# KIT-MBS/pydca

Measured on AMD Instinct MI355X. Metric: plmDCA L-BFGS iterations/s (L=500 N=50000 q=21), higher is better.
Workload: dtype f32

## Files before the change

pydca_amd/csrc/lbfgs_kernels.h:

```cpp
#pragma once

#include "dca_internal.h"
#include "plm_plan.h"
#include "vec_kernels.h"

namespace {

template <bool DD> struct DotAcc;
template <> struct DotAcc<false> {
    double hi = 0.0;
    static constexpr double lo = 0.0;
    __device__ __forceinline__ void add(double a, double b) { hi += a * b; }
    __device__ __forceinline__ void wave_reduce() { for (int off = 32; off > 0; off >>= 1) hi += __shfl_down(hi, off); }
};
template <> struct DotAcc<true> {
    double hi = 0.0, lo = 0.0;
    __device__ __forceinline__ void add(double a, double b) { dd_add(hi, lo, __dmul_rn(a, b)); }
    __device__ __forceinline__ void wave_reduce() { dd_wave_reduce(hi, lo); }
};
template <int NV>
__device__ __forceinline__ void dot_block_store(double (*red)[2 * NV], int nv, double* __restrict__ partials, unsigned grid = 0)
{
    __syncthreads();
    if ((int)threadIdx.x < nv) {
// ... 174 lines not shown
        if (e < (size_t)L * Q) {
            T sv[5], yv[5];
#pragma unroll
            for (int k = 0; k < 5; ++k) { sv[k] = static_cast<const T*>(P.s[k])[e]; yv[k] = static_cast<const T*>(P.y[k])[e]; }
            const T dv = compose_elem(c, g[e], sv, yv);
            d[e] = dv;
            const T v = one * dv;
            xt[e] = x[e] + v;
        }
        return;
    }
    const int blk = ((int)blockIdx.x & ~63) | (((int)blockIdx.x & 7) << 3) | (((int)blockIdx.x >> 3) & 7);
    if (blk >= pairBlocks) return;
    const int i0 = (blk / numJC) * TI, j0 = (blk % numJC) * JC;
    const int j1 = min(j0 + JC, L);
    if (j1 <= i0 + 1) return;
    if (tid == 0) {
        int pre = 0;
        for (int ii = 0; ii < TI; ++ii) {
            const int i = i0 + ii, jlo = max(j0, i + 1);
            const int cnt = jlo < j1 ? (j1 - jlo) * Q2 : 0;
            const size_t before = (size_t)L * (L - 1) / 2 - (size_t)(L - i) * (L - i - 1) / 2;
            const size_t lo = cnt ? (size_t)L * Q + (before + (size_t)(jlo - i - 1)) * Q2 : 0;
            sLo[ii] = lo; sCnt[ii] = cnt; sPre[ii] = pre;
            pre += cnt ? (int)((lo + cnt + VEC - 1) / VEC - lo / VEC) : 0;
        }
        sPre[TI] = pre;
    }
    __syncthreads();
    const int total = sPre[TI];
    for (int idx = tid; idx < total; idx += kFusedStepThreads) {
        int ii = 0;
        while (idx >= sPre[ii + 1]) ++ii;
        const size_t lo = sLo[ii], hi = lo + (size_t)sCnt[ii];
        const size_t iv = lo / VEC + (size_t)(idx - sPre[ii]);
        const Pack<T> pg = ldp_at(g, iv); const Pack<T> px = ldp_at(x, iv);
        Pack<T> psk[5]; Pack<T> pyk[5];
#pragma unroll
        for (int k = 0; k < 5; ++k) { psk[k] = ldp_at(static_cast<const T*>(P.s[k]), iv); pyk[k] = ldp_at(static_cast<const T*>(P.y[k]), iv); }
        Pack<T> od, ox;
#pragma unroll
        for (int u = 0; u < VEC; ++u) {
            T sv[5], yv[5];
#pragma unroll
            for (int k = 0; k < 5; ++k) { sv[k] = psk[k].v[u]; yv[k] = pyk[k].v[u]; }
            od.v[u] = compose_elem(c, pg.v[u], sv, yv);
            const T v = one * od.v[u];
            ox.v[u] = px.v[u] + v;
        }
        const size_t e0 = iv * VEC;
        T* const dst = tile + (size_t)(ii * JC + (max(j0, i0 + ii + 1) - j0)) * Q2;
        if (e0 >= lo && e0 + VEC <= hi) {
            stp_at(d, iv, od); stp_at(xt, iv, ox);
#pragma unroll
            for (int u = 0; u < VEC; ++u) dst[e0 + u - lo] = ox.v[u];
        } else {
#pragma unroll
            for (int u = 0; u < VEC; ++u) {
                const size_t e = e0 + u;
                if (e >= lo && e < hi) { d[e] = od.v[u]; xt[e] = ox.v[u]; dst[e - lo] = ox.v[u]; }
            }
        }
    }
    __syncthreads();
    {
        constexpr int WD = JC * Q;
        int row = tid / WD, col = tid % WD;
        while (row < TI * Q) {
            const int ii = row / Q, jj = col / Q;
            const int i = i0 + ii, j = j0 + jj;
            if (j > i && j < j1) W[(size_t)(i0 * Q + row) * Cs + j0 * Q + col] = tile[row * Q + ii * ((JC - 1) * Q2) + col + jj * ((Q - 1) * Q)];
            row += kFusedStepThreads / WD; col += kFusedStepThreads % WD;
            if (col >= WD) { col -= WD; ++row; }
        }
    }
    {
        constexpr int WD = TI * Q;
        int row = tid / WD, col = tid % WD;
        while (row < JC * Q) {
            const int jj = row / Q, ii = col / Q;
            const int i = i0 + ii, j = j0 + jj;
            if (j > i && j < j1) W[(size_t)(j0 * Q + row) * Cs + i0 * Q + col] = tile[col * Q + ii * ((JC - 1) * Q2) + row + jj * ((Q - 1) * Q)];
            row += kFusedStepThreads / WD; col += kFusedStepThreads % WD;
            if (col >= WD) { col -= WD; ++row; }
        }
    }
}

__global__ __launch_bounds__(256)
void vec_final_kernel(const double* __restrict__ partials, int nb, int nk, double* __restrict__ out)
{
    __shared__ double redHi[256], redLo[256];
    const int k = blockIdx.x;
    double hi = 0.0, lo = 0.0;
    for (int b = threadIdx.x; b < nb; b += blockDim.x) dd_add2(hi, lo, partials[2 * ((size_t)k * nb + b)], partials[2 * ((size_t)k * nb + b) + 1]);
    dd_block_reduce(hi, lo, redHi, redLo);
    if (threadIdx.x == 0) out[k] = hi + lo;
}

__global__ __launch_bounds__(256)
void dd_sum_chunks_kernel(const double* __restrict__ parts, int n, double* __restrict__ out)
{
    __shared__ double redHi[256], redLo[256];
    const int chunk = (n + gridDim.x - 1) / gridDim.x;
    const int lo_ = blockIdx.x * chunk, hi_ = min(n, lo_ + chunk);
    double hi = 0.0, lo = 0.0;
    for (int b = lo_ + threadIdx.x; b < hi_; b += blockDim.x) dd_add2(hi, lo, parts[2 * (size_t)b], parts[2 * (size_t)b + 1]);
    dd_block_reduce(hi, lo, redHi, redLo);
    if (threadIdx.x == 0) { out[2 * blockIdx.x] = hi; out[2 * blockIdx.x + 1] = lo; }
}
__global__ __launch_bounds__(1024)
void dd_sum_final_kernel(const double* __restrict__ A, int nA, const double* __restrict__ B, int nB, double* __restrict__ out)
{
    __shared__ double redHi[1024], redLo[1024];
    double hi = 0.0, lo = 0.0;
    for (int b = threadIdx.x; b < nA; b += blockDim.x) dd_add2(hi, lo, A[2 * (size_t)b], A[2 * (size_t)b + 1]);
    for (int b = threadIdx.x; b < nB; b += blockDim.x) dd_add2(hi, lo, B[2 * (size_t)b], B[2 * (size_t)b + 1]);
    dd_block_reduce(hi, lo, redHi, redLo);
    if (threadIdx.x == 0) out[0] = hi + lo;
}

template <typename T>
__global__ __launch_bounds__(kVecThreads)
void vec_dot3_fx_kernel(const T* __restrict__ a, const T* __restrict__ b, const T* __restrict__ c, size_t n, double* __restrict__ partials,
                        const double* __restrict__ fxParts, int nFxParts, double* __restrict__ fxChunks)
{
    if (blockIdx.x >= (unsigned)kVecBlocks) {
        __shared__ double redHi[256], redLo[256];
        const int blk = (int)blockIdx.x - kVecBlocks;
        const int chunk = (nFxParts + kSumStageBlocks - 1) / kSumStageBlocks;
        const int lo_ = blk * chunk, hi_ = min(nFxParts, lo_ + chunk);
        double hi = 0.0, lo = 0.0;
        for (int p = lo_ + threadIdx.x; p < hi_; p += blockDim.x) dd_add2(hi, lo, fxParts[2 * (size_t)p], fxParts[2 * (size_t)p + 1]);
        dd_block_reduce(hi, lo, redHi, redLo);
        if (threadIdx.x == 0) { fxChunks[2 * blk] = hi; fxChunks[2 * blk + 1] = lo; }
        return;
    }
    __shared__ double red[kVecThreads / 64][6];
    DotAcc<sizeof(T) == 8> s0, s1, s2;
    DCA_VEC_LOOP_G(n, a, kVecBlocks,
        const Pack<T> pa = ldp_at(a + head_, iv); const Pack<T> pb = ldp_at(b + head_, iv); const Pack<T> pc = ldp_at(c + head_, iv);
        _Pragma("unroll") for (int k = 0; k < VEC; ++k) {
            const double av = pa.v[k]; const double bv = pb.v[k]; const double cv = pc.v[k];
            s0.add(av, bv); s1.add(cv, cv); s2.add(av, av);
        },
        { const double av = a[i]; const double bv = b[i]; const double cv = c[i]; s0.add(av, bv); s1.add(cv, cv); s2.add(av, av); })
    s0.wave_reduce(); s1.wave_reduce(); s2.wave_reduce();
    if ((threadIdx.x & 63) == 0) {
        double* r = red[threadIdx.x >> 6];
        r[0] = s0.hi; r[1] = s0.lo; r[2] = s1.hi; r[3] = s1.lo; r[4] = s2.hi; r[5] = s2.lo;
    }
    dot_block_store<3>(red, 3, partials, kVecBlocks);
}
__global__ __launch_bounds__(1024)
void vec_final_fx_kernel(const double* __restrict__ partials, int nb, int nk, double* __restrict__ out,
                         const double* __restrict__ A, int nA, const double* __restrict__ B, int nB, double* __restrict__ fxOut)
{
    __shared__ double redHi[1024], redLo[1024];
    const int k = blockIdx.x;
    double hi = 0.0, lo = 0.0;
    if (k < nk) {
        constexpr int NT = 256;
        if ((int)threadIdx.x < NT) {
            for (int b = threadIdx.x; b < nb; b += NT) dd_add2(hi, lo, partials[2 * ((size_t)k * nb + b)], partials[2 * ((size_t)k * nb + b) + 1]);
            redHi[threadIdx.x] = hi;
            redLo[threadIdx.x] = lo;
        }
        __syncthreads();
        for (int st = NT / 2; st > 0; st >>= 1) {
            if ((int)threadIdx.x < st) dd_add2(redHi[threadIdx.x], redLo[threadIdx.x], redHi[threadIdx.x + st], redLo[threadIdx.x + st]);
            __syncthreads();
        }
        if (threadIdx.x == 0) out[k] = redHi[0] + redLo[0];
        return;
    }
    for (int b = threadIdx.x; b < nA; b += blockDim.x) dd_add2(hi, lo, A[2 * (size_t)b], A[2 * (size_t)b + 1]);
    for (int b = threadIdx.x; b < nB; b += blockDim.x) dd_add2(hi, lo, B[2 * (size_t)b], B[2 * (size_t)b + 1]);
    dd_block_reduce(hi, lo, redHi, redLo);
    if (threadIdx.x == 0) fxOut[0] = hi + lo;
}

}
```

pydca_amd/csrc/plm_engine.hip:

```cpp
#include <algorithm>
#include <chrono>
#include <cmath>

#include "dca_internal.h"
#include "more_thuente.h"
#include "vec_kernels.h"
#include "plm_plan.h"
#include "plm_stages.h"
#include "lbfgs_kernels.h"

namespace {

static_assert(kPlanXcds == kNumXcd, "the planner deals strips to this many XCDs");

#ifdef DCA_ROUND_ABLATE
__global__ void round_to_f32_kernel(double* __restrict__ p, size_t n)
{
    for (size_t i = blockIdx.x * (size_t)blockDim.x + threadIdx.x; i < n; i += (size_t)gridDim.x * blockDim.x) p[i] = (double)(float)p[i];
}
inline int round_stage_mask() { const char* e = getenv("DCA_ROUND_F32_STAGES"); return e ? atoi(e) : 0; }
#define DCA_ROUND_STAGE(bit, ptr, count)                                                                             \
    do {                                                                                                             \
        if constexpr (sizeof(T) == 8)                                                                                \
            if (round_stage_mask() & (bit))                                                                          \
                hipLaunchKernelGGL(round_to_f32_kernel, dim3(2048), dim3(256), 0, ctx->stream, reinterpret_cast<double*>(ptr), (size_t)(count)); \
    } while (0)
#else
#define DCA_ROUND_STAGE(bit, ptr, count) do { } while (0)
#endif

template <typename T>
struct PlmEngine : PlmEngineBase {
    dca_ctx* ctx;
    int N, L, q, Ls;
    double lambda_h = 0, lambda_J = 0;
    int carry_mode = DCA_CARRY_CHUNKED, halo = 0, add_reg = 1;
    bool configured = false;
    PlmPlan plan;
    PlmKnobs knobs;

    T *dx = nullptr, *dg = nullptr, *dxp = nullptr, *dgp = nullptr, *dd = nullptr;
    T* dS[5] = {nullptr, nullptr, nullptr, nullptr, nullptr};
    T* dY[5] = {nullptr, nullptr, nullptr, nullptr, nullptr};
    T *dWt = nullptr, *dSR = nullptr, *dR = nullptr, *dG = nullptr, *dw = nullptr;
    LbfgsDev* dLb = nullptr;
    uint16_t* dXL = nullptr;
    uint16_t* dXT2 = nullptr;
    PairIJ* dPairs = nullptr;
    double *dFxPart = nullptr, *dRegPart = nullptr, *dVecPart = nullptr;
    double *dColPart = nullptr, *dColSum = nullptr;
    double* dColChunk = nullptr;
    bool stripRequested = false, strips = false, stripEmulate = false;
    int sWorld = 1, sRank = 0;
    T *dGrecv = nullptr, *dXsend = nullptr, *dXrecv = nullptr;
    template <typename F> void each_buffer(F f)
    {
        f(dx); f(dg); f(dxp); f(dgp); f(dd);
        for (int i = 0; i < 5; ++i) { f(dS[i]); f(dY[i]); }
        f(dWt); f(dSR); f(dR); f(dG); f(dw); f(dLb); f(dXL); f(dXT2); f(dPairs); f(dFxPart); f(dRegPart); f(dVecPart);
        f(dColPart); f(dColSum); f(dColChunk); f(dGrecv); f(dXsend); f(dXrecv);
    }
    int strip_cs(int r) const { return plm_strip_cs(plan.siteB, q, r); }
    size_t owned_lo(int r) const { return plm_owned_lo(plan.siteB, L, q, r); }
    size_t owned_hi(int r) const { return plm_owned_hi(plan.siteB, L, q, r); }
    bool lbfgs_alloc = false;
    bool deferFx = false, fxPending = false;
    size_t vlo = 0, vn = 0, Ppad = 0;
    dca_comm_hook comm = nullptr;
    void* comm_user = nullptr;
    int comm_rank = 0, comm_world = 0;

    struct {
        bool begun = false, finished = false;
        int status = 0, k = 1, end = 0, iters = 0, evals = 0, max_iterations = 0, verbose = 0;
        double fx = 0, step = 0, xnorm = 0, gnorm = 0, seconds = 0;
        double last_step = 0;
        double dginit = 0;
        bool dginit_on_device = false;
        bool trial_ready = false;
    } o;

    explicit PlmEngine(dca_ctx* c) : ctx(c), N(c->N), L(c->L), q(c->q), Ls(c->Ls) {}

    template <typename U> int dalloc(U** p, size_t n)
    {
        HIP_TRY(dca_dev_malloc(reinterpret_cast<void**>(p), std::max<size_t>(n, 1) * sizeof(U)));
        return DCA_OK;
    }
    void freeall() { each_buffer([](auto*& p) { dca_dev_free(p); p = nullptr; }); }
    ~PlmEngine() override { freeall(); }

    void weights_changed() override { configured = false; o = decltype(o)(); }

    int configure(double lh, double lJ, int cmode, int chunk_, int warm_, int halo_, int add_reg_) override
    {
        if (q != 21 && q != 5) { dca_set_error("plmDCA kernels are built for q = 21 (protein) and q = 5 (RNA); got %d", q); return DCA_ERR_ARG; }
        if (!ctx->have_weights) { dca_set_error("weights must be computed or set before dca_plm_configure"); return DCA_ERR_STATE; }
        if (halo_ < 0 || halo_ >= N) { dca_set_error("halo out of range"); return DCA_ERR_ARG; }
        if (L > 65535) { dca_set_error("L too large"); return DCA_ERR_ARG; }
        configured = false;
        lambda_h = lh; lambda_J = lJ; carry_mode = cmode; halo = halo_; add_reg = add_reg_;
        strips = stripRequested && ctx->comm && ctx->comm_world > 1;
        stripRequested = false;
        sWorld = strips ? ctx->comm_world : 1;
        sRank = strips ? ctx->comm_rank : 0;
#ifdef DCA_ROUND_ABLATE
        stripEmulate = false;
        if (const char* e = getenv("DCA_STRIP_EMULATE")) {
            int er = 0, ew = 1;
            if (sscanf(e, "%d,%d", &er, &ew) == 2 && ew > 1 && er >= 0 && er < ew) { strips = true; stripEmulate = true; sRank = er; sWorld = ew; }
        }
#endif
        if (sWorld > kMaxStripRanks || (strips && sWorld > L)) { dca_set_error("column strips: too many ranks for %d sites", L); return DCA_ERR_ARG; }
        if (strips && (halo || hook || comm)) { dca_set_error("column strips take the whole alignment and no hooks"); return DCA_ERR_ARG; }
        knobs = PlmKnobs::from_env();
        PlmShape shape;
        shape.N = N; shape.L = L; shape.q = q; shape.elemBytes = (int)sizeof(T); shape.halo = halo; shape.chunkArg = chunk_; shape.warmArg = warm_;
        shape.carryMode = carry_mode; shape.stripWorld = sWorld; shape.stripRank = sRank; shape.strips = strips;
        plan = plm_make_plan(shape, knobs, PlmKernelShapes{{logits_seq_per_wg(5), logits_seq_per_wg(21), logits_seq_per_wg(kPairQ)},
                                                           {logits_jt(5), logits_jt(21), logits_jt(kPairQ)}});
        const int Lq = L * q, JT = plan.JT;
        const size_t npairs = (size_t)L * (L - 1) / 2;

        freeall();
        lbfgs_alloc = false;
        o = decltype(o)();

        DCA_TRY(dalloc(&dx, plan.P + kVecPad)); DCA_TRY(dalloc(&dg, plan.P + kVecPad));
        DCA_TRY(dalloc(&dWt, (size_t)plan.Wrows * plan.Cs));
        DCA_TRY(dalloc(&dSR, (size_t)N * plan.Cs));
        DCA_TRY(dalloc(&dR, (size_t)(N + kNC) * plan.Cs));
        HIP_TRY(hipMemsetAsync(dR, 0, (size_t)(N + kNC) * plan.Cs * sizeof(T), ctx->stream));
        DCA_TRY(dalloc(&dG, plan.num_slabs() * plan.slab_elems()));
        DCA_TRY(dalloc(&dw, N));
        DCA_TRY(dalloc(&dXL, (size_t)ceil_div(plan.gUnits, JT) * JT * plan.Npad));
        DCA_TRY(dalloc(&dXT2, (size_t)plan.gUnits * plan.NT));
        DCA_TRY(dalloc(&dPairs, npairs));
        DCA_TRY(dalloc(&dFxPart, 2 * (size_t)plan.nFxPart));
        DCA_TRY(dalloc(&dRegPart, 2 * (size_t)(plan.nRegPart + kSumStageBlocks)));
        DCA_TRY(dalloc(&dVecPart, 2 * 27 * kVecBlocks));
        HIP_TRY(hipMemsetAsync(dRegPart, 0, 2 * (size_t)(plan.nRegPart + kSumStageBlocks) * sizeof(double), ctx->stream));
        HIP_TRY(hipMemsetAsync(dFxPart, 0, 2 * (size_t)plan.nFxPart * sizeof(double), ctx->stream));
        if (sizeof(T) == 8) {
            DCA_TRY(dalloc(&dColPart, 2 * (size_t)kColSumRowBlocks * Lq));
            if (q == 5) DCA_TRY(dalloc(&dColChunk, 2 * (size_t)plan.numScanChunks * Lq));
            DCA_TRY(dalloc(&dColSum, (size_t)Lq));
        }
        if (strips) { DCA_TRY(dalloc(&dGrecv, plan.grecvOff[sWorld])); DCA_TRY(dalloc(&dXsend, plan.xsendOff[sWorld])); DCA_TRY(dalloc(&dXrecv, plan.xrecvOff[sWorld])); }

        HIP_TRY(hipMemsetAsync(dx, 0, (plan.P + kVecPad) * sizeof(T), ctx->stream));
        HIP_TRY(hipMemsetAsync(dg, 0, (plan.P + kVecPad) * sizeof(T), ctx->stream));
        vlo = 0; vn = plan.P; Ppad = plan.P;
        if (strips) {
            native_mode = 4;
            vlo = plan.oLo; vn = plan.oHi - plan.oLo;
        } else if (native_mode == 4) {
            native_mode = 0;
        }
        if (native_mode == 2 || native_mode == 3) {
            if (!ctx->comm) native_mode = 0;
            else DCA_TRY(set_slices(ctx->comm_rank, ctx->comm_world));
        } else if (comm) {
            DCA_TRY(set_slices(comm_rank, comm_world));
        }
        if (native_mode == 1 && !ctx->comm) native_mode = 0;
        HIP_TRY(hipMemsetAsync(dWt, 0, (size_t)plan.Wrows * plan.Cs * sizeof(T), ctx->stream));
        HIP_TRY(hipMemsetAsync(dG, 0, plan.num_slabs() * plan.slab_elems() * sizeof(T), ctx->stream));

        std::vector<PairIJ> hp(npairs);
        {
            size_t k = 0;
            for (int i = 0; i < L - 1; ++i) for (int j = i + 1; j < L; ++j) hp[k++] = PairIJ{(uint16_t)i, (uint16_t)j};
        }
        HIP_TRY(hipMemcpyAsync(dPairs, hp.data(), npairs * sizeof(PairIJ), hipMemcpyHostToDevice, ctx->stream));
        HIP_TRY(hipStreamSynchronize(ctx->stream));

        std::vector<T> hw(N);
        {
            std::vector<double> wd(N);
            HIP_TRY(hipMemcpy(wd.data(), ctx->dWd, (size_t)N * sizeof(double), hipMemcpyDeviceToHost));
            if (ctx->have_counts) {
                std::vector<uint32_t> cnt(N);
                HIP_TRY(hipMemcpy(cnt.data(), ctx->dCounts, (size_t)N * sizeof(uint32_t), hipMemcpyDeviceToHost));
                for (int n = 0; n < N; ++n) hw[n] = (T)1 / (T)cnt[n];
            } else {
                for (int n = 0; n < N; ++n) hw[n] = (T)wd[n];
            }
        }
        HIP_TRY(hipMemcpy(dw, hw.data(), (size_t)N * sizeof(T), hipMemcpyHostToDevice));

        if (plan.pairs) {
            hipLaunchKernelGGL(plm_build_pair_states_kernel, dim3(ceil_div(plan.Npad, 256), ceil_div(plan.gUnits, JT) * JT), dim3(256), 0,
                               ctx->stream, ctx->dX, dXL, N, plan.Npad, L, Ls, 0, 0x2000u);
            hipLaunchKernelGGL(plm_build_pair_states_kernel, dim3(ceil_div(plan.NT, 256), plan.gUnits), dim3(256), 0, ctx->stream,
                               ctx->dX, dXT2, N, plan.NT, L, Ls, halo, 0x9000u);
            HIP_TRY(hipGetLastError());
            HIP_TRY(hipStreamSynchronize(ctx->stream));
        } else {
            hipLaunchKernelGGL(plm_build_logit_states_kernel, dim3(ceil_div(plan.Npad, 256), ceil_div(L, JT) * JT), dim3(256), 0,
                               ctx->stream, ctx->dX, dXL, N, plan.Npad, L, Ls);
            hipLaunchKernelGGL(plm_build_states_kernel, dim3(ceil_div(plan.NT, 256), L), dim3(256), 0, ctx->stream,
                               ctx->dX, dXT2, N, L, Ls, halo, plan.NT);
            HIP_TRY(hipGetLastError());
            HIP_TRY(hipStreamSynchronize(ctx->stream));
        }
        configured = true;
        return DCA_OK;
    }

    int configure_strips(double lh, double lJ, int cmode, int chunk_, int warm_) override
    {
        if (!ctx->comm) { dca_set_error("column strips need a communicator: dca_comm_init first"); return DCA_ERR_STATE; }
        if (o.begun && !o.finished) { dca_set_error("the decomposition cannot change during an optimisation"); return DCA_ERR_STATE; }
        const auto hook0 = hook; const auto hookUser0 = hook_user; const auto comm0 = comm; const auto commUser0 = comm_user;
        const int commRank0 = comm_rank, commWorld0 = comm_world;
        hook = nullptr; hook_user = nullptr; comm = nullptr; comm_user = nullptr; comm_rank = comm_world = 0;
        stripRequested = true;
        const int rc = configure(lh, lJ, cmode, chunk_, warm_, 0, 1);
        stripRequested = false;
        if (rc != DCA_OK) { hook = hook0; hook_user = hookUser0; comm = comm0; comm_user = commUser0; comm_rank = commRank0; comm_world = commWorld0; strips = false; }
        return rc;
    }

    int init_x() override
    {
        if (!configured) { dca_set_error("dca_plm_configure first"); return DCA_ERR_STATE; }
        std::vector<T> hw(N);
        HIP_TRY(hipMemcpy(hw.data(), dw, (size_t)N * sizeof(T), hipMemcpyDeviceToHost));
        T meff = 0;
        for (int n = 0; n < N; ++n) meff += hw[n];
        std::vector<T> h((size_t)L * q, (T)0);
        const uint8_t* X = dca_host_msa(ctx);
        if (!X) return DCA_ERR_HIP;
        for (int n = 0; n < N; ++n)
            for (int i = 0; i < L; ++i) h[(size_t)i * q + X[(size_t)n * L + i]] += hw[n];
        for (int i = 0; i < L; ++i) {
            T* hi = h.data() + (size_t)i * q;
            for (int a = 0; a < q; ++a) hi[a] /= meff;
            for (int a = 0; a < q; ++a) hi[a] = std::log(hi[a] * meff + (T)1);
            T s = 0;
            for (int a = 0; a < q; ++a) s += hi[a];
            const T av = s / (T)q;
            for (int a = 0; a < q; ++a) hi[a] -= av;
        }
        o.trial_ready = false;
        HIP_TRY(hipMemsetAsync(dx, 0, plan.P * sizeof(T), ctx->stream));
        HIP_TRY(hipMemcpyAsync(dx, h.data(), h.size() * sizeof(T), hipMemcpyHostToDevice, ctx->stream));
        HIP_TRY(hipStreamSynchronize(ctx->stream));
        return DCA_OK;
    }

    template <typename U> int upload(const U* src, T* dst)
    {
        std::vector<T> tmp(plan.P);
        for (size_t i = 0; i < plan.P; ++i) tmp[i] = (T)src[i];
        HIP_TRY(hipMemcpy(dst, tmp.data(), plan.P * sizeof(T), hipMemcpyHostToDevice));
        return DCA_OK;
    }
    template <typename U> int download(const T* src, U* dst)
    {
        std::vector<T> tmp(plan.P);
        HIP_TRY(hipStreamSynchronize(ctx->stream));
        HIP_TRY(hipMemcpy(tmp.data(), src, plan.P * sizeof(T), hipMemcpyDeviceToHost));
        for (size_t i = 0; i < plan.P; ++i) dst[i] = (U)tmp[i];
        return DCA_OK;
    }
    int set_x(const void* x, int dtype) override
    {
        if (!configured) { dca_set_error("dca_plm_configure first"); return DCA_ERR_STATE; }
        o.trial_ready = false;
        if (dtype == DCA_F32) return upload(static_cast<const float*>(x), dx);
        if (dtype == DCA_F64) return upload(static_cast<const double*>(x), dx);
        return DCA_ERR_ARG;
    }
    int get_x(void* x, int dtype) override
    {
        if (!configured) return DCA_ERR_STATE;
        if (native_mode == 4 && !stripEmulate) DCA_TRY(strip_allgather(dx));
        if (dtype == DCA_F32) return download(dx, static_cast<float*>(x));
        if (dtype == DCA_F64) return download(dx, static_cast<double*>(x));
        return DCA_ERR_ARG;
    }
    int get_g(void* g, int dtype) override
    {
        if (!configured) return DCA_ERR_STATE;
        DCA_TRY(gather_vector(dg));
        if (dtype == DCA_F32) return download(dg, static_cast<float*>(g));
        if (dtype == DCA_F64) return download(dg, static_cast<double*>(g));
        return DCA_ERR_ARG;
    }

    template <int Q> int launch_eval(bool w_ready)
    {
// ... 150 lines not shown
        if (native_mode == 4) return stripEmulate ? DCA_OK : strip_allgather(v);
        return do_comm(DCA_COMM_ALL_GATHER, v, Ppad, (int)sizeof(T) * 8, "all-gather");
    }
    int publish_x()
    {
        if (native_mode == 4) return stripEmulate ? DCA_OK : exchange_x();
        return gather_vector(dx);
    }

    int exchange_x()
    {
        const int dt = (int)sizeof(T) * 8;
        const size_t q2 = (size_t)q * q;
        for (int r = sRank + 1; r < sWorld; ++r) {
            const int ni = plan.siteB[r + 1] - plan.siteB[r];
            hipLaunchKernelGGL((strip_pairs_copy_kernel<T, true>), dim3((unsigned)(plan.Lloc * ni)), dim3(64), 0, ctx->stream, dx, dXsend + plan.xsendOff[r], L, q, plan.cS0, plan.cS1, plan.siteB[r], plan.siteB[r + 1]);
        }
        DCA_TRY(dca_comm_p2p_begin(ctx));
        int rc = DCA_OK;
        if (sRank == 0) { for (int r = 1; r < sWorld && rc == DCA_OK; ++r) rc = dca_comm_p2p_send(ctx, dx + (size_t)plan.siteB[r] * q, (size_t)(plan.siteB[r + 1] - plan.siteB[r]) * q, dt, r); }
        else rc = dca_comm_p2p_recv(ctx, dx + (size_t)plan.cS0 * q, (size_t)plan.Lloc * q, dt, 0);
        for (int r = sRank + 1; r < sWorld && rc == DCA_OK; ++r) rc = dca_comm_p2p_send(ctx, dXsend + plan.xsendOff[r], (size_t)plan.Lloc * (plan.siteB[r + 1] - plan.siteB[r]) * q2, dt, r);
        for (int r = 0; r < sRank && rc == DCA_OK; ++r) rc = dca_comm_p2p_recv(ctx, dXrecv + plan.xrecvOff[r], (size_t)(plan.siteB[r + 1] - plan.siteB[r]) * plan.Lloc * q2, dt, r);
        const int rc2 = dca_comm_p2p_end(ctx);
        if (rc != DCA_OK) return rc;
        DCA_TRY(rc2);
        for (int r = 0; r < sRank; ++r) {
            const int nj = plan.siteB[r + 1] - plan.siteB[r];
            hipLaunchKernelGGL((strip_pairs_copy_kernel<T, false>), dim3((unsigned)(nj * plan.Lloc)), dim3(64), 0, ctx->stream, dx, dXrecv + plan.xrecvOff[r], L, q, plan.siteB[r], plan.siteB[r + 1], plan.cS0, plan.cS1);
        }
        HIP_TRY(hipGetLastError());
        return DCA_OK;
    }
    int exchange_g()
    {
        const int dt = (int)sizeof(T) * 8;
        DCA_TRY(dca_comm_p2p_begin(ctx));
        int rc = DCA_OK;
        for (int r = 0; r < sRank && rc == DCA_OK; ++r)
            rc = dca_comm_p2p_send(ctx, dG + (size_t)plan.siteB[r] * q * plan.Cs, (size_t)(plan.siteB[r + 1] - plan.siteB[r]) * q * plan.Cs, dt, r);
        for (int r = sRank + 1; r < sWorld && rc == DCA_OK; ++r)
            rc = dca_comm_p2p_recv(ctx, dGrecv + plan.grecvOff[r], (size_t)plan.Lloc * q * strip_cs(r), dt, r);
        if (rc == DCA_OK) {
            if (sRank > 0) rc = dca_comm_p2p_send(ctx, dg + (size_t)plan.cS0 * q, (size_t)plan.Lloc * q, dt, 0);
            else for (int r = 1; r < sWorld && rc == DCA_OK; ++r) rc = dca_comm_p2p_recv(ctx, dg + (size_t)plan.siteB[r] * q, (size_t)(plan.siteB[r + 1] - plan.siteB[r]) * q, dt, r);
        }
        const int rc2 = dca_comm_p2p_end(ctx);
        if (rc != DCA_OK) return rc;
        return rc2;
    }
    int strip_allgather(T* v)
    {
        const int dt = (int)sizeof(T) * 8;
        DCA_TRY(dca_comm_p2p_begin(ctx));
        int rc = DCA_OK;
        for (int k = 1; k < sWorld && rc == DCA_OK; ++k) {
            const int to = (sRank + k) % sWorld, from = (sRank - k + sWorld) % sWorld;
            rc = dca_comm_p2p_send(ctx, v + plan.oLo, plan.oHi - plan.oLo, dt, to);
            if (rc == DCA_OK) rc = dca_comm_p2p_recv(ctx, v + owned_lo(from), owned_hi(from) - owned_lo(from), dt, from);
        }
        const int rc2 = dca_comm_p2p_end(ctx);
        if (rc != DCA_OK) return rc;
        return rc2;
    }
    int bm_source(void** x) override
    {
        if (!configured) { dca_set_error("dca_plm_configure first"); return DCA_ERR_STATE; }
        if (o.begun && !o.finished) { dca_set_error("an L-BFGS run is in progress: dca_plm_lbfgs_end first"); return DCA_ERR_STATE; }
        if (strips || native_mode == 4) { dca_set_error("Boltzmann learning runs on one GPU: configured for column strips"); return DCA_ERR_STATE; }
        if (comm || hook || native_mode != 0) {
            dca_set_error("Boltzmann learning runs on one GPU: vector sharding, a reduce / comm hook or a native-comm mode is set");
            return DCA_ERR_STATE;
        }
        *x = dx;
        return DCA_OK;
    }
    int potts_source(PottsSource* out, bool one_gpu_only) override
    {
        if (!configured) { dca_set_error("dca_plm_configure first"); return DCA_ERR_STATE; }
        if (one_gpu_only) {
            if (strips || native_mode == 4) { dca_set_error("AIS, conditional sampling and the ascent run on one GPU: configured for column strips"); return DCA_ERR_STATE; }
            if (comm || hook || native_mode != 0) {
                dca_set_error("AIS, conditional sampling and the ascent run on one GPU: vector sharding, a reduce / comm hook or a native-comm mode is set");
                return DCA_ERR_STATE;
            }
        } else if (native_mode == 4 && !stripEmulate) {
            DCA_TRY(strip_allgather(dx));
        }
        *out = PottsSource{dx, 0, (int)sizeof(T) * 8, nullptr, L, q, 0};
        return DCA_OK;
    }
    int set_vector_sharding(int rank, int world, dca_comm_hook h, void* user) override
    {
        if (!configured) { dca_set_error("dca_plm_configure first"); return DCA_ERR_STATE; }
        if (o.begun && !o.finished) { dca_set_error("vector sharding cannot change during an optimisation"); return DCA_ERR_STATE; }
        if (strips) { dca_set_error("configured for column strips: dca_plm_configure again first"); return DCA_ERR_STATE; }
        if (native_mode >= 2) native_mode = 0;
        if (!h || world < 1) { vlo = 0; vn = plan.P; Ppad = plan.P; comm = nullptr; comm_user = nullptr; comm_rank = comm_world = 0; return DCA_OK; }
        DCA_TRY(set_slices(rank, world));
        comm = h; comm_user = user; comm_rank = rank; comm_world = world;
        return DCA_OK;
    }
    int set_slices(int rank, int world)
    {
        if (rank < 0 || rank >= world || world > 64) { dca_set_error("bad rank / world"); return DCA_ERR_ARG; }
        const size_t slice = (plan.P + (size_t)world * 4 - 1) / ((size_t)world * 4) * 4;
        if (slice * world > plan.P + kVecPad) { dca_set_error("world too large for the vector padding"); return DCA_ERR_ARG; }
        Ppad = slice * world;
        vlo = slice * rank;
        vn = vlo >= plan.P ? 0 : std::min(slice, plan.P - vlo);
        return DCA_OK;
    }
    bool configured_for_comm() const override { return configured; }
    int set_native_comm(int mode) override
    {
        if (!configured) { dca_set_error("dca_plm_configure first"); return DCA_ERR_STATE; }
        if (o.begun && !o.finished) { dca_set_error("the exchange scheme cannot change during an optimisation"); return DCA_ERR_STATE; }
        if (mode != 0 && !ctx->comm) { dca_set_error("no communicator: dca_comm_init first"); return DCA_ERR_STATE; }
        if (mode == 4) { dca_set_error("the column-strip decomposition is set up by dca_plm_configure_strips"); return DCA_ERR_ARG; }
        if (mode < 0 || mode > 3) return DCA_ERR_ARG;
        if (strips) {
            if (mode != 0) { dca_set_error("configured for column strips: dca_plm_configure again first"); return DCA_ERR_STATE; }
            configured = false; strips = false; native_mode = 0; o = decltype(o)();
            return DCA_OK;
        }
        if (mode >= 2) DCA_TRY(set_slices(ctx->comm_rank, ctx->comm_world));
        else { vlo = 0; vn = plan.P; Ppad = plan.P; }
        comm = nullptr; comm_user = nullptr; comm_rank = comm_world = 0;
        if (mode != 0) { hook = nullptr; hook_user = nullptr; }
        native_mode = mode;
        return DCA_OK;
    }

    int read_scalars(int n)
    {
        HIP_TRY(hipMemcpyAsync(ctx->hScal, ctx->dScal, (size_t)n * sizeof(double), hipMemcpyDeviceToHost, ctx->stream));
        HIP_TRY(hipStreamSynchronize(ctx->stream));
        return DCA_OK;
    }

    int gradient(double* fx_out) override
    {
        o.trial_ready = false;
        DCA_TRY(evaluate_async());
        DCA_TRY(reduce_scalars(0, 1));
        DCA_TRY(gather_vector(dg));
        DCA_TRY(read_scalars(1));
        if (fx_out) *fx_out = ctx->hScal[0];
        return DCA_OK;
    }

    void v_neg(T* d, const T* g) { hipLaunchKernelGGL(vec_neg_kernel<T>, dim3(kVecBlocks), dim3(kVecThreads), 0, ctx->stream, d + vlo, g + vlo, vn); }
    void v_step(T* x, const T* xp, double stp, const T* d) { hipLaunchKernelGGL(vec_step_kernel<T>, dim3(kVecBlocks), dim3(kVecThreads), 0, ctx->stream, x + vlo, xp + vlo, (T)stp, d + vlo, vn); }
    int eval_scalars(double* fx, double* gd, double* xx, double* gg)
    {
        if (fxPending) {
            double* const fxChunks = dRegPart + 2 * (size_t)plan.nRegPart;
            hipLaunchKernelGGL(vec_dot3_fx_kernel<T>, dim3(kVecBlocks + kSumStageBlocks), dim3(kVecThreads), 0, ctx->stream, dg + vlo, dd + vlo, dx + vlo, vn, dVecPart,
                               dRegPart, plan.nRegPart, fxChunks);
            hipLaunchKernelGGL(vec_final_fx_kernel, dim3(3 + 1), dim3(1024), 0, ctx->stream, dVecPart, kVecBlocks, 3, ctx->dScal + 1,
                               fxChunks, kSumStageBlocks, dFxPart, plan.nFxPart, ctx->dScal);
            fxPending = false;
        } else {
            hipLaunchKernelGGL(vec_dot3_kernel<T>, dim3(kVecBlocks), dim3(kVecThreads), 0, ctx->stream, dg + vlo, dd + vlo, dx + vlo, vn, dVecPart);
            hipLaunchKernelGGL(vec_final_kernel, dim3(3), dim3(256), 0, ctx->stream, dVecPart, kVecBlocks, 3, ctx->dScal + 1);
        }
        DCA_TRY(reduce_scalars(0, 4));
        DCA_TRY(read_scalars(kSlotDginit + 1));
        *fx = ctx->hScal[0]; *gd = ctx->hScal[1]; *xx = ctx->hScal[2]; *gg = ctx->hScal[3];
        if (o.dginit_on_device) { o.dginit = ctx->hScal[kSlotDginit]; o.dginit_on_device = false; }
        return DCA_OK;
    }

    int lbfgs_begin(int max_iterations, int verbose) override
    {
        if (!configured) { dca_set_error("dca_plm_configure first"); return DCA_ERR_STATE; }
        if (!lbfgs_alloc) {
            DCA_TRY(dalloc(&dxp, plan.P + kVecPad)); DCA_TRY(dalloc(&dgp, plan.P + kVecPad)); DCA_TRY(dalloc(&dd, plan.P + kVecPad));
            for (int i = 0; i < 5; ++i) { DCA_TRY(dalloc(&dS[i], plan.P + kVecPad)); DCA_TRY(dalloc(&dY[i], plan.P + kVecPad)); }
            HIP_TRY(hipMemsetAsync(dxp, 0, (plan.P + kVecPad) * sizeof(T), ctx->stream));
            HIP_TRY(hipMemsetAsync(dgp, 0, (plan.P + kVecPad) * sizeof(T), ctx->stream));
            HIP_TRY(hipMemsetAsync(dd, 0, (plan.P + kVecPad) * sizeof(T), ctx->stream));
            lbfgs_alloc = true;
        }
        for (int i = 0; i < 5; ++i) {
            HIP_TRY(hipMemsetAsync(dS[i], 0, (plan.P + kVecPad) * sizeof(T), ctx->stream));
            HIP_TRY(hipMemsetAsync(dY[i], 0, (plan.P + kVecPad) * sizeof(T), ctx->stream));
        }
        if (!dLb) HIP_TRY(dca_dev_malloc(reinterpret_cast<void**>(&dLb), sizeof(LbfgsDev)));
        HIP_TRY(hipMemsetAsync(dLb, 0, sizeof(LbfgsDev), ctx->stream));
        o = decltype(o)();
        o.max_iterations = max_iterations;
        o.verbose = verbose;
        auto t0 = std::chrono::steady_clock::now();
        DCA_TRY(evaluate_async(true));
        v_neg(dd, dg);
        double fx, gd, xx, gg;
        DCA_TRY(eval_scalars(&fx, &gd, &xx, &gg));
        o.fx = fx;
        o.xnorm = std::sqrt(xx); o.gnorm = std::sqrt(gg);
        const double xn = std::max(o.xnorm, 1.0);
        o.begun = true;
        if (o.gnorm / xn <= 1e-3) { o.status = LB_ALREADY_MINIMIZED; o.finished = true; }
        o.step = 1.0 / std::sqrt(gg);
        o.dginit = -gg;
        o.seconds += std::chrono::duration<double>(std::chrono::steady_clock::now() - t0).count();
        return DCA_OK;
    }

    int line_search(double* stp, double* f, double* xx, double* gg, int* rc_hip)
    {
        const MtParams params{1e-4, 0.9, 1e-16, 1e-20, 1e20, 5};
        const bool deferred = o.dginit_on_device;
        bool first = true;
        const int ls = mt_line_search(params, stp, f, &o.dginit, deferred, [&](double t, double* ft, double* dgt) {
            const bool ready = o.trial_ready && first && t == 1.0 && fused_step_ok();
            o.trial_ready = false; first = false;
            if (!ready) {
                v_step(dx, dxp, t, dd);
                DCA_ROUND_STAGE(32, dx, plan.P);
            }
            DCA_TRY(publish_x());
            DCA_TRY(evaluate_async(true, ready));
            return eval_scalars(ft, dgt, xx, gg);
        }, rc_hip);
        if (deferred && ls == LB_INCREASEGRADIENT) o.evals -= 1;
        return ls;
    }

    void lbfgs_end() override { o = decltype(o)(); }
    bool fused_step_ok() const
    {
#ifdef DCA_ROUND_ABLATE
        if (round_stage_mask()) return false;
#endif
        return knobs.fuseStep != 0 && native_mode == 0 && !hook && !comm && !strips && !stripEmulate && vlo == 0 && vn == plan.P &&
               plan.cS0 == 0 && plan.cS1 == L;
    }
    template <int Q> void launch_fused_step(const VecPtrs5& ptrs)
    {
        const int numJC = ceil_div(L, fused_step_jc(Q)), pairBlocks = ceil_div(L, fused_step_ti(Q, (int)sizeof(T))) * numJC;
        const size_t lds = (size_t)fused_step_ti(Q, (int)sizeof(T)) * fused_step_jc(Q) * Q * Q * sizeof(T);
        hipLaunchKernelGGL((lbfgs_dir_trial_expand_kernel<T, Q>), dim3((unsigned)(ceil_div(pairBlocks, 64) * 64 + ceil_div(L * Q, kFusedStepThreads))), dim3(kFusedStepThreads), lds,
                           ctx->stream, dd, dxp, dWt, dx, dg, ptrs, &dLb->cf, L, plan.Cs, numJC, pairBlocks);
    }
    int lbfgs_iterate(int iterations, dca_plm_stats* st) override
    {
        if (!o.begun) { dca_set_error("dca_plm_lbfgs_begin first"); return DCA_ERR_STATE; }
        auto t0 = std::chrono::steady_clock::now();
        constexpr int M = 5;
        for (int it = 0; it < iterations && !o.finished; ++it) {
            std::swap(dx, dxp);
            std::swap(dg, dgp);
            double xx = 0, gg = 0;
            int rc = 0;
            const int ls = line_search(&o.step, &o.fx, &xx, &gg, &rc);
            if (rc) return rc;
            if (ls < 0) {
                std::swap(dx, dxp);
                std::swap(dg, dgp);
                o.trial_ready = false;
                o.status = ls; o.finished = true;
                break;
            }
            o.xnorm = std::sqrt(xx); o.gnorm = std::sqrt(gg);
            o.iters = o.k;
            o.last_step = o.step;
            if (o.verbose) {
                fprintf(stderr, "Iteration %d:\n", o.k);
                fprintf(stderr, "fx = %f, xnorm = %f, gnorm = %f, step = %f\n\n", o.fx, o.xnorm, o.gnorm, o.step);
            }
            const double xn = std::max(o.xnorm, 1.0);
            if (o.gnorm / xn <= 1e-3) { o.status = 0; o.finished = true; break; }
            if (o.max_iterations != 0 && o.max_iterations < o.k + 1) { o.status = LB_MAXIMUMITERATION; o.finished = true; break; }

            const int e = o.end;
            VecPtrs5 ptrs;
            for (int i = 0; i < M; ++i) { ptrs.s[i] = dS[i] + vlo; ptrs.y[i] = dY[i] + vlo; }
            {
                ScopedKernelClock kc(ctx, "lbfgs_vec");
                auto gram = [&](auto slot) {
                    hipLaunchKernelGGL((vec_diff_gram_kernel<T, decltype(slot)::value>), dim3(kVecBlocks), dim3(kVecThreads), 0, ctx->stream, ptrs, dS[e] + vlo, dY[e] + vlo,
                                       dx + vlo, dxp + vlo, dg + vlo, dgp + vlo, vn, dVecPart);
                };
                switch (e) {
                case 0: gram(std::integral_constant<int, 0>()); break;
                case 1: gram(std::integral_constant<int, 1>()); break;
                case 2: gram(std::integral_constant<int, 2>()); break;
                case 3: gram(std::integral_constant<int, 3>()); break;
                default: gram(std::integral_constant<int, 4>()); break;
                }
                hipLaunchKernelGGL(vec_final_kernel, dim3(27), dim3(256), 0, ctx->stream, dVecPart, kVecBlocks, 27, ctx->dScal + 1);
            }
            DCA_TRY(reduce_scalars(1, 27));
            const int bound = (M <= o.k) ? M : o.k;
            ++o.k;
            o.end = (o.end + 1) % M;
            {
                ScopedKernelClock kc(ctx, "lbfgs_vec");
                hipLaunchKernelGGL(lbfgs_two_loop_kernel, dim3(1), dim3(64), 0, ctx->stream, ctx->dScal, dLb, e, o.end, bound, gg);
                if (fused_step_ok()) {
                    if (q == 21) launch_fused_step<21>(ptrs); else launch_fused_step<5>(ptrs);
                    o.trial_ready = true;
                } else {
                    hipLaunchKernelGGL(vec_compose_kernel<T>, dim3(kVecBlocks), dim3(kVecThreads), 0, ctx->stream, dd + vlo, dg + vlo, ptrs, &dLb->cf, vn);
                    DCA_ROUND_STAGE(64, dd, plan.P);
                }
                o.dginit_on_device = true;
            }
            o.step = 1.0;
        }
        HIP_TRY(hipStreamSynchronize(ctx->stream));
        o.seconds += std::chrono::duration<double>(std::chrono::steady_clock::now() - t0).count();
        if (st) {
            st->status = o.status; st->iterations = o.iters; st->evaluations = o.evals; st->finished = o.finished ? 1 : 0;
            st->fx = o.fx; st->xnorm = o.xnorm; st->gnorm = o.gnorm; st->step = o.iters ? o.last_step : o.step; st->seconds = o.seconds;
        }
        return DCA_OK;
    }

    int scores(int apc, double* out) override
    {
        if (!configured) return DCA_ERR_STATE;
        if (native_mode == 4 && !stripEmulate) DCA_TRY(strip_allgather(dx));
        const size_t npairs = (size_t)L * (L - 1) / 2;
        double* dOut = nullptr;
        HIP_TRY(dca_dev_malloc(reinterpret_cast<void**>(&dOut), npairs * sizeof(double)));
        int rc = dca_fn_scores(ctx, dx, 0, (int)sizeof(T) * 8, L, q, 0, apc, dOut);
        if (rc == DCA_OK) {
            hipError_t e = hipStreamSynchronize(ctx->stream);
            if (e == hipSuccess) e = hipMemcpy(out, dOut, npairs * sizeof(double), hipMemcpyDeviceToHost);
            if (e != hipSuccess) { dca_set_error("copy scores: %s", hipGetErrorString(e)); rc = DCA_ERR_HIP; }
        }
        dca_dev_free(dOut);
        return rc;
    }
    int pair_couplings(const int* pairs, int npairs, int shift, double* out) override
    {
        if (!configured) return DCA_ERR_STATE;
        if (native_mode == 4 && !stripEmulate) DCA_TRY(strip_allgather(dx));
        return dca_pair_blocks(ctx, dx, 0, (int)sizeof(T) * 8, L, q, 0, pairs, npairs, shift, out);
    }

    int di_scores(const double* reg_fi, int apc, double* out) override
    {
        if (!configured) return DCA_ERR_STATE;
        if (native_mode == 4 && !stripEmulate) DCA_TRY(strip_allgather(dx));
        const size_t npairs = (size_t)L * (L - 1) / 2;
        double *dOut = nullptr, *dFi = nullptr;
        HIP_TRY(dca_dev_malloc(reinterpret_cast<void**>(&dOut), npairs * sizeof(double)));
        if (dca_dev_malloc(reinterpret_cast<void**>(&dFi), (size_t)L * q * sizeof(double)) != hipSuccess) { dca_dev_free(dOut); return DCA_ERR_NOMEM; }
        int rc = DCA_OK;
        if (hipMemcpy(dFi, reg_fi, (size_t)L * q * sizeof(double), hipMemcpyHostToDevice) != hipSuccess) rc = DCA_ERR_HIP;
        if (rc == DCA_OK) rc = dca_di_scores(ctx, dx, 0, (int)sizeof(T) * 8, dFi, L, q, 0, apc, dOut);
        if (rc == DCA_OK) {
            hipError_t e = hipStreamSynchronize(ctx->stream);
            if (e == hipSuccess) e = hipMemcpy(out, dOut, npairs * sizeof(double), hipMemcpyDeviceToHost);
            if (e != hipSuccess) { dca_set_error("copy DI scores: %s", hipGetErrorString(e)); rc = DCA_ERR_HIP; }
        }
        dca_dev_free(dOut); dca_dev_free(dFi);
        return rc;
    }
};

}

PlmEngineBase* dca_make_plm_engine(dca_ctx* ctx)
{
    if (ctx->precision == DCA_F64) return new PlmEngine<double>(ctx);
    return new PlmEngine<float>(ctx);
}
```

Baseline: 62.13.

## Fuse L-BFGS diff/gram pass into first line-search scalar reduction kernel

```diff
diff --git a/pydca_amd/csrc/lbfgs_kernels.h b/pydca_amd/csrc/lbfgs_kernels.h
--- a/pydca_amd/csrc/lbfgs_kernels.h
+++ b/pydca_amd/csrc/lbfgs_kernels.h
@@ -350,6 +350,74 @@
     }
     dot_block_store<3>(red, 3, partials, kVecBlocks);
 }
+template <typename T, int E>
+__global__ __launch_bounds__(kVecThreads)
+void vec_dot3_fx_gram_kernel(VecPtrs5 P, T* __restrict__ se, T* __restrict__ ye, const T* __restrict__ x, const T* __restrict__ xp,
+                             const T* __restrict__ g, const T* __restrict__ gp, const T* __restrict__ d, size_t n,
+                             double* __restrict__ dotPartials, double* __restrict__ gramPartials,
+                             const double* __restrict__ fxParts, int nFxParts, double* __restrict__ fxChunks)
+{
+    if (blockIdx.x >= (unsigned)kVecBlocks) {
+        __shared__ double redHi[256], redLo[256];
+        const int blk = (int)blockIdx.x - kVecBlocks;
+        const int chunk = (nFxParts + kSumStageBlocks - 1) / kSumStageBlocks;
+        const int lo_ = blk * chunk, hi_ = min(nFxParts, lo_ + chunk);
+        double hi = 0.0, lo = 0.0;
+        for (int p = lo_ + threadIdx.x; p < hi_; p += blockDim.x) dd_add2(hi, lo, fxParts[2 * (size_t)p], fxParts[2 * (size_t)p + 1]);
+        dd_block_reduce(hi, lo, redHi, redLo);
+        if (threadIdx.x == 0) { fxChunks[2 * blk] = hi; fxChunks[2 * blk + 1] = lo; }
+        return;
+    }
+    __shared__ double red3[kVecThreads / 64][6];
+    __shared__ double red[kVecThreads / 64][54];
+    DotAcc<sizeof(T) == 8> s0, s1, s2;
+    DotAcc<sizeof(T) == 8> acc[27];
+    DCA_VEC_LOOP_G(n, se, kVecBlocks,
+        const Pack<T> px = ldp_at(x + head_, iv); const Pack<T> pxp = ldp_at(xp + head_, iv); const Pack<T> pg = ldp_at(g + head_, iv); const Pack<T> pgp = ldp_at(gp + head_, iv);
+        const Pack<T> pd = ldp_at(d + head_, iv);
+        Pack<T> psk[5]; Pack<T> pyk[5];
+        _Pragma("unroll") for (int k = 0; k < 5; ++k)
+            if (k != E) { psk[k] = ldp_at(static_cast<const T*>(P.s[k]) + head_, iv); pyk[k] = ldp_at(static_cast<const T*>(P.y[k]) + head_, iv); }
+        _Pragma("unroll") for (int k = 0; k < VEC; ++k) {
+            const double av = pg.v[k]; const double bv = pd.v[k]; const double cv = px.v[k];
+            s0.add(av, bv); s1.add(cv, cv); s2.add(av, av);
+        }
+        Pack<T> pse; Pack<T> pye;
+        _Pragma("unroll") for (int u = 0; u < VEC; ++u) {
+            pse.v[u] = px.v[u] - pxp.v[u]; pye.v[u] = pg.v[u] - pgp.v[u];
+            acc[0].add((double)pye.v[u], (double)pse.v[u]); acc[1].add((double)pye.v[u], (double)pye.v[u]);
+        }
+        psk[E] = pse; pyk[E] = pye;
+        stp_at(se + head_, iv, pse); stp_at(ye + head_, iv, pye);
+        _Pragma("unroll") for (int k = 0; k < 5; ++k) {
+            _Pragma("unroll") for (int u = 0; u < VEC; ++u) {
+                const double gv = pg.v[u]; const double sev = pse.v[u]; const double yev = pye.v[u];
+                const double sk = psk[k].v[u]; const double yk = pyk[k].v[u];
+                acc[2 + k].add(sk, gv); acc[7 + k].add(yk, gv); acc[12 + k].add(sev, yk); acc[17 + k].add(yev, sk); acc[22 + k].add(yev, yk);
+            }
+        },
+        { const double av = g[i]; const double bv = d[i]; const double cv = x[i]; s0.add(av, bv); s1.add(cv, cv); s2.add(av, av);
+          const T sev_ = x[i] - xp[i]; const T yev_ = g[i] - gp[i]; se[i] = sev_; ye[i] = yev_;
+          const double gv = g[i]; const double sev = sev_; const double yev = yev_;
+          acc[0].add(yev, sev); acc[1].add(yev, yev);
+          _Pragma("unroll") for (int k = 0; k < 5; ++k) {
+              const double sk = k == E ? sev : (double)static_cast<const T*>(P.s[k])[i]; const double yk = k == E ? yev : (double)static_cast<const T*>(P.y[k])[i];
+              acc[2 + k].add(sk, gv); acc[7 + k].add(yk, gv); acc[12 + k].add(sev, yk); acc[17 + k].add(yev, sk); acc[22 + k].add(yev, yk);
+          } })
+    const int lane = threadIdx.x & 63, wv = threadIdx.x >> 6;
+    s0.wave_reduce(); s1.wave_reduce(); s2.wave_reduce();
+    if (lane == 0) {
+        double* r = red3[wv];
+        r[0] = s0.hi; r[1] = s0.lo; r[2] = s1.hi; r[3] = s1.lo; r[4] = s2.hi; r[5] = s2.lo;
+    }
+#pragma unroll
+    for (int v = 0; v < 27; ++v) {
+        acc[v].wave_reduce();
+        if (lane == 0) { red[wv][2 * v] = acc[v].hi; red[wv][2 * v + 1] = acc[v].lo; }
+    }
+    dot_block_store<3>(red3, 3, dotPartials, kVecBlocks);
+    dot_block_store<27>(red, 27, gramPartials, kVecBlocks);
+}
 __global__ __launch_bounds__(1024)
 void vec_final_fx_kernel(const double* __restrict__ partials, int nb, int nk, double* __restrict__ out,
                          const double* __restrict__ A, int nA, const double* __restrict__ B, int nB, double* __restrict__ fxOut)
diff --git a/pydca_amd/csrc/plm_engine.hip b/pydca_amd/csrc/plm_engine.hip
--- a/pydca_amd/csrc/plm_engine.hip
+++ b/pydca_amd/csrc/plm_engine.hip
@@ -38,6 +38,7 @@
     bool configured = false;
     PlmPlan plan;
     PlmKnobs knobs;
+    int fuseTail = 1;
 
     T *dx = nullptr, *dg = nullptr, *dxp = nullptr, *dgp = nullptr, *dd = nullptr;
     T* dS[5] = {nullptr, nullptr, nullptr, nullptr, nullptr};
@@ -48,6 +49,7 @@
     uint16_t* dXT2 = nullptr;
     PairIJ* dPairs = nullptr;
     double *dFxPart = nullptr, *dRegPart = nullptr, *dVecPart = nullptr;
+    double* dGramPart = nullptr;
     double *dColPart = nullptr, *dColSum = nullptr;
     double* dColChunk = nullptr;
     bool stripRequested = false, strips = false, stripEmulate = false;
@@ -57,7 +59,7 @@
     {
         f(dx); f(dg); f(dxp); f(dgp); f(dd);
         for (int i = 0; i < 5; ++i) { f(dS[i]); f(dY[i]); }
-        f(dWt); f(dSR); f(dR); f(dG); f(dw); f(dLb); f(dXL); f(dXT2); f(dPairs); f(dFxPart); f(dRegPart); f(dVecPart);
+        f(dWt); f(dSR); f(dR); f(dG); f(dw); f(dLb); f(dXL); f(dXT2); f(dPairs); f(dFxPart); f(dRegPart); f(dVecPart); f(dGramPart);
         f(dColPart); f(dColSum); f(dColChunk); f(dGrecv); f(dXsend); f(dXrecv);
     }
     int strip_cs(int r) const { return plm_strip_cs(plan.siteB, q, r); }
@@ -78,6 +80,7 @@
         double dginit = 0;
         bool dginit_on_device = false;
         bool trial_ready = false;
+        bool tail_ready = false;
     } o;
 
     explicit PlmEngine(dca_ctx* c) : ctx(c), N(c->N), L(c->L), q(c->q), Ls(c->Ls) {}
@@ -114,6 +117,7 @@
         if (sWorld > kMaxStripRanks || (strips && sWorld > L)) { dca_set_error("column strips: too many ranks for %d sites", L); return DCA_ERR_ARG; }
         if (strips && (halo || hook || comm)) { dca_set_error("column strips take the whole alignment and no hooks"); return DCA_ERR_ARG; }
         knobs = PlmKnobs::from_env();
+        { const char* e = getenv("DCA_PLM_FUSE_TAIL"); fuseTail = (e && atoi(e) == 0) ? 0 : 1; }
         PlmShape shape;
         shape.N = N; shape.L = L; shape.q = q; shape.elemBytes = (int)sizeof(T); shape.halo = halo; shape.chunkArg = chunk_; shape.warmArg = warm_;
         shape.carryMode = carry_mode; shape.stripWorld = sWorld; shape.stripRank = sRank; shape.strips = strips;
@@ -139,6 +143,7 @@
         DCA_TRY(dalloc(&dFxPart, 2 * (size_t)plan.nFxPart));
         DCA_TRY(dalloc(&dRegPart, 2 * (size_t)(plan.nRegPart + kSumStageBlocks)));
         DCA_TRY(dalloc(&dVecPart, 2 * 27 * kVecBlocks));
+        DCA_TRY(dalloc(&dGramPart, 2 * 27 * kVecBlocks));
         HIP_TRY(hipMemsetAsync(dRegPart, 0, 2 * (size_t)(plan.nRegPart + kSumStageBlocks) * sizeof(double), ctx->stream));
         HIP_TRY(hipMemsetAsync(dFxPart, 0, 2 * (size_t)plan.nFxPart * sizeof(double), ctx->stream));
         if (sizeof(T) == 8) {
@@ -595,9 +600,32 @@
 
     void v_neg(T* d, const T* g) { hipLaunchKernelGGL(vec_neg_kernel<T>, dim3(kVecBlocks), dim3(kVecThreads), 0, ctx->stream, d + vlo, g + vlo, vn); }
     void v_step(T* x, const T* xp, double stp, const T* d) { hipLaunchKernelGGL(vec_step_kernel<T>, dim3(kVecBlocks), dim3(kVecThreads), 0, ctx->stream, x + vlo, xp + vlo, (T)stp, d + vlo, vn); }
-    int eval_scalars(double* fx, double* gd, double* xx, double* gg)
-    {
-        if (fxPending) {
+    int eval_scalars(double* fx, double* gd, double* xx, double* gg, bool with_tail = false)
+    {
+        if (fxPending && with_tail) {
+            double* const fxChunks = dRegPart + 2 * (size_t)plan.nRegPart;
+            VecPtrs5 ptrs;
+            for (int i = 0; i < 5; ++i) { ptrs.s[i] = dS[i] + vlo; ptrs.y[i] = dY[i] + vlo; }
+            const int e = o.end;
+            auto tail = [&](auto slot) {
+                hipLaunchKernelGGL((vec_dot3_fx_gram_kernel<T, decltype(slot)::value>), dim3(kVecBlocks + kSumStageBlocks), dim3(kVecThreads), 0, ctx->stream, ptrs,
+                                   dS[e] + vlo, dY[e] + vlo, dx + vlo, dxp + vlo, dg + vlo, dgp + vlo, dd + vlo, vn, dVecPart, dGramPart, dRegPart, plan.nRegPart, fxChunks);
+            };
+            {
+                ScopedKernelClock kc(ctx, "lbfgs_vec");
+                switch (e) {
+                case 0: tail(std::integral_constant<int, 0>()); break;
+                case 1: tail(std::integral_constant<int, 1>()); break;
+                case 2: tail(std::integral_constant<int, 2>()); break;
+                case 3: tail(std::integral_constant<int, 3>()); break;
+                default: tail(std::integral_constant<int, 4>()); break;
+                }
+            }
+            hipLaunchKernelGGL(vec_final_fx_kernel, dim3(3 + 1), dim3(1024), 0, ctx->stream, dVecPart, kVecBlocks, 3, ctx->dScal + 1,
+                               fxChunks, kSumStageBlocks, dFxPart, plan.nFxPart, ctx->dScal);
+            fxPending = false;
+            o.tail_ready = true;
+        } else if (fxPending) {
             double* const fxChunks = dRegPart + 2 * (size_t)plan.nRegPart;
             hipLaunchKernelGGL(vec_dot3_fx_kernel<T>, dim3(kVecBlocks + kSumStageBlocks), dim3(kVecThreads), 0, ctx->stream, dg + vlo, dd + vlo, dx + vlo, vn, dVecPart,
                                dRegPart, plan.nRegPart, fxChunks);
@@ -658,14 +686,15 @@
         bool first = true;
         const int ls = mt_line_search(params, stp, f, &o.dginit, deferred, [&](double t, double* ft, double* dgt) {
             const bool ready = o.trial_ready && first && t == 1.0 && fused_step_ok();
-            o.trial_ready = false; first = false;
+            const bool tail = first && fused_tail_ok();
+            o.trial_ready = false; o.tail_ready = false; first = false;
             if (!ready) {
                 v_step(dx, dxp, t, dd);
                 DCA_ROUND_STAGE(32, dx, plan.P);
             }
             DCA_TRY(publish_x());
             DCA_TRY(evaluate_async(true, ready));
-            return eval_scalars(ft, dgt, xx, gg);
+            return eval_scalars(ft, dgt, xx, gg, tail);
         }, rc_hip);
         if (deferred && ls == LB_INCREASEGRADIENT) o.evals -= 1;
         return ls;
@@ -679,6 +708,13 @@
 #endif
         return knobs.fuseStep != 0 && native_mode == 0 && !hook && !comm && !strips && !stripEmulate && vlo == 0 && vn == plan.P &&
                plan.cS0 == 0 && plan.cS1 == L;
+    }
+    bool fused_tail_ok() const
+    {
+#ifdef DCA_ROUND_ABLATE
+        if (round_stage_mask()) return false;
+#endif
+        return fuseTail != 0 && native_mode == 0 && !hook && !comm && !strips && !stripEmulate && vlo == 0 && vn == plan.P;
     }
     template <int Q> void launch_fused_step(const VecPtrs5& ptrs)
     {
@@ -698,6 +734,8 @@
             double xx = 0, gg = 0;
             int rc = 0;
             const int ls = line_search(&o.step, &o.fx, &xx, &gg, &rc);
+            const bool tailDone = o.tail_ready;
+            o.tail_ready = false;
             if (rc) return rc;
             if (ls < 0) {
                 std::swap(dx, dxp);
@@ -720,7 +758,7 @@
             const int e = o.end;
             VecPtrs5 ptrs;
             for (int i = 0; i < M; ++i) { ptrs.s[i] = dS[i] + vlo; ptrs.y[i] = dY[i] + vlo; }
-            {
+            if (!tailDone) {
                 ScopedKernelClock kc(ctx, "lbfgs_vec");
                 auto gram = [&](auto slot) {
                     hipLaunchKernelGGL((vec_diff_gram_kernel<T, decltype(slot)::value>), dim3(kVecBlocks), dim3(kVecThreads), 0, ctx->stream, ptrs, dS[e] + vlo, dY[e] + vlo,
@@ -741,6 +779,7 @@
             o.end = (o.end + 1) % M;
             {
                 ScopedKernelClock kc(ctx, "lbfgs_vec");
+                if (tailDone) hipLaunchKernelGGL(vec_final_kernel, dim3(27), dim3(256), 0, ctx->stream, dGramPart, kVecBlocks, 27, ctx->dScal + 1);
                 hipLaunchKernelGGL(lbfgs_two_loop_kernel, dim3(1), dim3(64), 0, ctx->stream, ctx->dScal, dLb, e, o.end, bound, gg);
                 if (fused_step_ok()) {
                     if (q == 21) launch_fused_step<21>(ptrs); else launch_fused_step<5>(ptrs);
```

Result: no change. 61.54 (-0.9%).
